# welcomyou/sherpa-vietnamese-asr

Measured on AMD Instinct MI355X. Metric: audio-sec/sec (xRT) Zipformer-68M offline decode, higher is better.
Workload: dtype bf16; 1 GPU; zipformer-68m greedy_search, batched planner chunks, 1 h per GPU; model=zipformer-68m, weights=greedy-calibrated, chunks_per_gpu=121, batch_pipeline=True, encoder_frames_per_gpu=98813

## Files before the change

include/zasr.h:

```cpp
#ifndef ZASR_H_
#define ZASR_H_

#include <stdint.h>

#ifdef __cplusplus
extern "C" {
#endif

typedef struct zasr_recognizer zasr_recognizer;
typedef struct zasr_result zasr_result;

enum {
  ZASR_OK = 0,
  ZASR_ERR_INVALID = 1,
  ZASR_ERR_NOT_FOUND = 2,
  ZASR_ERR_RUNTIME = 3,
};

enum {
  ZASR_PRECISION_FP32 = 0,
  ZASR_PRECISION_BF16 = 1,
  ZASR_PRECISION_BF16_ENC = 2,
  ZASR_PRECISION_BF16X3 = 3,
  ZASR_PRECISION_BF16X6 = 4,
// ... 106 lines not shown
void zasr_vad_destroy(zasr_vad* h);
int zasr_vad_probs(zasr_vad* h, const float* audio, const int64_t* offsets,
                   const int64_t* lengths, int32_t n_files, int32_t auto_boost, float* probs);
int zasr_vad_probs_device(zasr_vad* h, const float* d_audio, const int64_t* offsets,
                          const int64_t* lengths, int32_t n_files, int32_t auto_boost,
                          float* d_probs, void* stream);
int32_t zasr_vad_last_passes(const zasr_vad* h);
int zasr_vad_window(zasr_vad* h, const float* input, const float* state, int32_t n, float* prob,
                    float* state_out);

int32_t zasr_vocab_size(const zasr_recognizer* h);
int32_t zasr_joiner_dim(const zasr_recognizer* h);
int zasr_model_routes(zasr_recognizer* h, char* buf, int64_t cap);
int zasr_fbank_set_mel_banks(zasr_recognizer* h, const float* banks, int32_t n_bins);
int zasr_selftest_launch(int32_t block_threads);
int zasr_selftest_gemm_h3r(int32_t M, int32_t K, int32_t N, int32_t epi, const float* A,
                           const float* W, const float* bias, float* C);
int zasr_selftest_ffn_h3(int32_t R, int32_t D, int32_t F, const float* Y, const float* W1,
                         const float* b1, const float* W2, const float* b2,
                         const float* byp_orig, const float* byp_scale, float* X);
int zasr_selftest_ffn_bf16(int32_t R, int32_t D, int32_t F, const float* W1, const float* b1,
                           const float* W2, const float* b2, const float* byp_orig,
                           const float* byp_scale, float* X, int32_t form);

int zasr_profile_enable(zasr_recognizer* h, int32_t on);
int zasr_profile_reset(zasr_recognizer* h);
int zasr_profile_report(zasr_recognizer* h, char* buf, int64_t cap);

const char* zasr_last_error(void);
const char* zasr_version(void);

#ifdef __cplusplus
}
#endif
#endif
```

sherpa-vietnamese-asr_amd/csrc/attn_kernels.hip:

```cpp
#include <mutex>
#include <string>
#include <type_traits>
#include <unordered_map>

#include "common.h"
#include "gemm.h"
#include "gemm_dev.h"
#include "kernels.h"

namespace zasr {


namespace {
constexpr int kKLd = 40;
constexpr int kPosPad = 160;

__device__ __forceinline__ float fexp2(float x) { return __builtin_amdgcn_exp2f(x); }

typedef float f32x2 __attribute__((ext_vector_type(2)));
typedef __bf16 bf16x2 __attribute__((ext_vector_type(2)));
__device__ __forceinline__ f32x2 pk_fma(f32x2 a, f32x2 b, f32x2 c) { return __builtin_elementwise_fma(a, b, c); }

typedef _Float16 f16x8a __attribute__((ext_vector_type(8)));
typedef _Float16 f16x2 __attribute__((ext_vector_type(2)));
__device__ __forceinline__ void mfma_h3s(const bf16x8 (&x)[2], const f16x8a& ys, const f16x8a& yh,
                                         const f16x8a& yl, f32x16& acc) {
// ... 18 lines not shown
    lp[q / 2] = lo;
  }
  ys = __builtin_bit_cast(f16x8a, sp);
  yl = __builtin_bit_cast(f16x8a, lp);
  const _Float16 k = (_Float16)(1.f / 2048.f);
  yh = ys * (f16x8a){k, k, k, k, k, k, k, k};
}

}

template <int MODE, int NP, int FMT = 0, int NF = 1>
__global__ __launch_bounds__(256) void attn_flash_kernel(AttnFlashArgs a) {
  constexpr bool SPLIT = NP > 1;
  constexpr bool P1 = FMT == 1;
  static_assert(FMT == 0 || NP == 2, "fp16 pieces: NP = 2");
  static_assert(MODE != 3 || NP == 1 || (NP == 2 && FMT == 1),
                "fused NonlinAttention: the bf16 and f16x3 modes");
  constexpr bool W0 = MODE == 0 || MODE == 3;
  using T = typename std::conditional<SPLIT, float, __bf16>::type;
  extern __shared__ float sPos[];
  __shared__ __attribute__((aligned(16))) __bf16 sK[NP][2][32 * kKLd];
  __shared__ __attribute__((aligned(16))) __bf16 sVt[NP][2][12 * kKLd];
  __shared__ __attribute__((aligned(16))) __bf16 sVn[NP][2][MODE == 3 ? NF * 32 * kKLd : 8];
  const int b = blockIdx.y;
  const int h = W0 ? 0 : blockIdx.z;
  const int fz = MODE == 3 ? blockIdx.z : 0;
  const int r0 = a.row_off[b];
  const int L = a.row_off[b + 1] - r0;
  const int i0b = blockIdx.x * 128;
  if (i0b >= L) return;
  const int H = a.H;
  const long ldq = 68L * H;
  const long ldv = 12L * H;
  const T* qkp = reinterpret_cast<const T*>(a.qkp);
  const int tid = threadIdx.x, lane = tid & 63, wid = tid >> 6;
  const int c = lane & 31, h2 = lane >> 5;
  const int i0 = i0b + 32 * wid;
  const bool live = i0 < L;
  const int i = i0 + c;
  const int ic = i < L ? i : L - 1;
  constexpr float kSc = SPLIT ? 1.4426950408889634f : 1.f;
  constexpr float kE = P1 ? 11.f : 0.f;

  {
    const int xlo = -(i0b + 127);
    const int n = L + kPosPad;
    const int rmax = 2 * a.pmax - 2;
    for (int t = tid; t < n; t += 256) {
      int row = xlo + t + a.pmax - 1;
      row = row < 0 ? 0 : (row > rmax ? rmax : row);
      const float4 v = *reinterpret_cast<const float4*>(a.pos_tab + (long)row * 4 * H + 4 * h);
      if constexpr (SPLIT) {
        sPos[t] = v.x;
// ... 483 lines not shown
  static std::mutex mu;
  static std::unordered_map<const void*, size_t> memo;
  std::lock_guard<std::mutex> g(mu);
  auto it = memo.find(fn);
  if (it != memo.end()) return it->second;
  hipFuncAttributes at{};
  ZASR_HIP_CHECK(hipFuncGetAttributes(&at, fn));
  return memo[fn] = at.sharedSizeBytes;
}

template <int MODE, int NP, int FMT, int NF>
static void launch_flash_one(const AttnFlashArgs& a, dim3 grid, size_t lds, hipStream_t st) {
  const void* fn = reinterpret_cast<const void*>(&attn_flash_kernel<MODE, NP, FMT, NF>);
  const size_t stat = kernel_static_lds(fn);
  if (lds + stat > kLdsPerCu)
    throw std::runtime_error("attention: sequence of " + std::to_string(a.max_len) +
                             " frames needs " + std::to_string(lds + stat) +
                             " B of LDS (positional stage + static staging), over the " +
                             std::to_string(kLdsPerCu) + " B of a gfx950 CU");
  ZASR_LAUNCH((attn_flash_kernel<MODE, NP, FMT, NF>), grid, dim3(256), lds, st, a);
}

template <int NP, int FMT = 0>
void launch_flash_np(const AttnFlashArgs& a, int mode, size_t lds, hipStream_t st) {
  const dim3 grid(cdiv(a.max_len, 128), a.nseq, mode == 0 ? 1 : a.H);
  if (mode == 0)
    launch_flash_one<0, NP, FMT, 1>(a, grid, lds, st);
  else if (mode == 1)
    launch_flash_one<1, NP, FMT, 1>(a, grid, lds, st);
  else
    launch_flash_one<2, NP, FMT, 1>(a, grid, lds, st);
}

void launch_attn_flash(const AttnFlashArgs& a, int mode, hipStream_t st) {
  if (a.nseq <= 0 || a.max_len <= 0) return;
  if (mode == 3) {
    ZASR_REQUIRE((a.pieces == 1 || a.pieces == kPiecesF16) && a.t1t && a.o8 && a.y && a.z &&
                     a.hid > 0 && a.hid % 4 == 0 && a.ldt % 8 == 0 && a.ldy % 4 == 0,
                 "attention mode 3: the bf16 or f16x3 mode, hid % 4 == 0");
    const size_t lds = (size_t)(a.max_len + kPosPad) * sizeof(float4);
    const int nft = cdiv(a.hid, 32);
    if (a.pieces == kPiecesF16) {
      const dim3 grid(cdiv(a.max_len, 128), a.nseq, cdiv(nft, 3));
      launch_flash_one<3, 2, 1, 3>(a, grid, lds, st);
      return;
    }
    const int nf = (nft % 5 == 0 || nft == 9) ? 5 : 6;
    const dim3 grid(cdiv(a.max_len, 128), a.nseq, cdiv(nft, nf));
    if (nf == 5)
      launch_flash_one<3, 1, 0, 5>(a, grid, lds, st);
    else
      launch_flash_one<3, 1, 0, 6>(a, grid, lds, st);
    return;
  }
  ZASR_REQUIRE(a.H % 2 == 0, "attention: the bf16 kernels need an even head count (16-byte q/k rows)");
  const size_t lds = (size_t)(a.max_len + kPosPad) * sizeof(float4);
  if (a.pieces == 1)
    launch_flash_np<1>(a, mode, lds, st);
  else if (a.pieces == 2)
    launch_flash_np<2>(a, mode, lds, st);
  else if (a.pieces == 3)
    launch_flash_np<3>(a, mode, lds, st);
  else if (a.pieces == kPiecesF16)
    launch_flash_np<2, 1>(a, mode, lds, st);
  else
    throw std::runtime_error("attention: pieces must be 1, 2, 3 or kPiecesF16");
}

__device__ __forceinline__ float4 h3_load4(const float* p) { return *reinterpret_cast<const float4*>(p); }
__device__ __forceinline__ float4 h3_load4(const __bf16* p) {
  const bf16x4 v = *reinterpret_cast<const bf16x4*>(p);
  return make_float4((float)v[0], (float)v[1], (float)v[2], (float)v[3]);
}

template <typename TH, int NP>
__global__ __launch_bounds__(256) void nonlin_prep_t_kernel(const TH* __restrict__ h3,
                                                            const int* __restrict__ off,
                                                            const int* __restrict__ o8,
                                                            const int* __restrict__ map, int R,
                                                            int hid, int R8,
                                                            __bf16* __restrict__ t1t) {
  __shared__ float tile[64][65];
  __shared__ int sRow[64];
  const int col0 = blockIdx.x * 64, c0 = blockIdx.y * 64;
  const int tid = threadIdx.x;
  if (tid < 64) {
    const int col = col0 + tid;
    int lo = 0, hi = map[R - 1];
    while (lo < hi) {
// ... 99 lines not shown
```

sherpa-vietnamese-asr_amd/csrc/engine.cpp:

```cpp
#include "engine.h"

#include <algorithm>
#include <cmath>
#include <cstring>
#include <deque>
#include <numeric>
#include <cstdlib>
#include <sstream>

#include "common.h"
#include "gemm.h"
#include "host_io.h"
#include "onnx_io.h"

namespace zasr {

namespace {
struct HwNode {
  int tok = -1;
  double tok_score = 0, node_score = 0, out_score = 0;
  bool is_end = false;
  std::vector<std::pair<int, int>> kids;
  int fail = 0, out = -1;
  int child(int t) const {
// ... 961 lines not shown
  m.len = len;
  m.off.assign(len.size() + 1, 0);
  for (size_t b = 0; b < len.size(); ++b) {
    m.off[b + 1] = m.off[b] + len[b];
    m.maxlen = std::max(m.maxlen, len[b]);
  }
  m.total = m.off.back();
  return m;
}
struct MetaPack {
  std::vector<char> bytes;
  size_t add(const void* p, size_t n) {
    size_t at = (bytes.size() + 15) & ~size_t(15);
    bytes.resize(at + n);
    if (n) std::memcpy(bytes.data() + at, p, n);
    return at;
  }
};
}

void Engine::layer_forward(const DStack& S, const DLayer& Ly, float* X, int R, const int* d_off,
                           const int* d_map,
                           const std::vector<int>& lens, const long* d_aoff,
                           const void* d_slices_nl, int maxL, const int* d_o8, int R8, bool orig_ready, bool last_layer) {
  const int d = S.d, h = S.h, B = (int)lens.size();
  const int hid = 3 * d / 4;
  float* O = ws<float>("ly_orig", (size_t)R * d);
  if (!orig_ready)
    ZASR_HIP_CHECK(hipMemcpyAsync(O, X, (size_t)R * d * sizeof(float), hipMemcpyDeviceToDevice, st_));
  const bool bf16 = precision_ == 1 || precision_ == 2;
  const int np = split_pieces();
  float* qkp = nullptr;
  float* A = nullptr;
  __bf16* A16 = nullptr;
  float* stats = nullptr;
  AttnFlashArgs fa{};
  if (bf16) {
    __bf16* qkp16 = ws<__bf16>("ly_qkp_h", (size_t)R * 68 * h);
    linear_h(Ly.attn_in, X, false, d, R, qkp16, true, 68 * h, EPI_NONE);
    A16 = ws<__bf16>("ly_attn_h", 1);
    stats = ws<float>("ly_attn_stats", (size_t)R * h);
    fa = AttnFlashArgs{qkp16, h, Ly.pos_tab, model_.pmax, d_off, d_aoff, B, maxL, A16,
                       nullptr, nullptr, stats, stats};
  } else if (np) {
    qkp = ws<float>("ly_qkp", (size_t)R * 68 * h);
    linear(Ly.attn_in, X, d, R, qkp, 68 * h, EPI_NONE);
    A = ws<float>("ly_attn", 1);
    stats = ws<float>("ly_attn_stats", (size_t)R * h);
    fa = AttnFlashArgs{qkp, h, Ly.pos_tab, model_.pmax, d_off, d_aoff, B, maxL, A,
                       nullptr, nullptr, stats, stats, np};
    if (np != kPiecesF16) {
      prof_begin("attn_softmax");
      launch_attn_flash(fa, 0, st_);
      prof_end();
    }
  } else {
    qkp = ws<float>("ly_qkp", (size_t)R * 68 * h);
    linear(Ly.attn_in, X, d, R, qkp, 68 * h, EPI_NONE);
    A = ws<float>("ly_attn", 1);
    stats = ws<float>("ly_attn_stats", (size_t)R * h * 2);
    AttnArgs a{qkp, h, Ly.pos_tab, model_.pmax, d_off, d_aoff, B, maxL, A, stats, 1};
    prof_begin("attn_softmax");
    launch_attn_softmax(a, st_);
    prof_end();
  }
  auto ff = [&](int k) {
    const DLin& fi = Ly.ff_in[k];
    const float* bo = (bf16 && k == 1) ? O : nullptr;
    const float* bs = (bf16 && k == 1) ? Ly.bypass_mid : nullptr;
    if (fi.wh && ffn_fused_supported(d) && (d < 256 || fi.wp)) {
      prof_begin("ffn_fused");
      launch_ffn_fused(X, R, d, fi.N, d < 256 ? fi.wh : fi.wp, fi.b,
                       d < 256 ? Ly.ff_out[k].wh : Ly.ff_out[k].wp, Ly.ff_out[k].b, st_, bo, bs);
      prof_end();
      return;
    }
// ... 2 lines not shown
      linear_h(fi, X, false, d, R, H, true, fi.N, EPI_SWOOSHL);
      linear_h(Ly.ff_out[k], H, true, fi.N, R, X, false, d, EPI_RESADD, bo, bs);
    } else if (fi.wp && np == kPiecesF16) {
      prof_begin("ffn_fused");
      launch_ffn_fused_h3(X, R, d, fi.N, fi.wp, fi.b, Ly.ff_out[k].wp, Ly.ff_out[k].b, st_,
                          k == 1 ? O : nullptr, k == 1 ? Ly.bypass_mid : nullptr);
      prof_end();
    } else {
      const bool byp = k == 1 && Ly.ff_out[k].wx != nullptr;
      float* H = ws<float>("ly_hid", (size_t)R * fi.N);
      linear(fi, X, d, R, H, fi.N, EPI_SWOOSHL);
      linear(Ly.ff_out[k], H, fi.N, R, X, d, EPI_RESADD, "enc_gemm", byp ? O : nullptr,
             byp ? Ly.bypass_mid : nullptr);
    }
  };
  auto self_attn = [&](int k) {
    if (bf16) {
      __bf16* vv = ws<__bf16>("ly_vv_h", (size_t)R * 12 * h);
      __bf16* oa = ws<__bf16>("ly_oa_h", (size_t)R * 12 * h);
      linear_h(Ly.sa_in[k], X, false, d, R, vv, true, 12 * h, EPI_NONE);
      AttnFlashArgs a = fa;
      a.v = vv;
      a.out = oa;
      prof_begin("attn_apply");
      launch_attn_flash(a, k == 0 ? 1 : 2, st_);
      prof_end();
      linear_h(Ly.sa_out[k], oa, true, 12 * h, R, X, false, d, EPI_RESADD);
      return;
    }
    float* vv = ws<float>("ly_vv", (size_t)R * 12 * h);
    float* oa = ws<float>("ly_oa", (size_t)R * 12 * h);
    linear(Ly.sa_in[k], X, d, R, vv, 12 * h, EPI_NONE);
    if (np) {
      AttnFlashArgs a = fa;
      a.v = vv;
      a.out = oa;
      prof_begin("attn_apply");
      launch_attn_flash(a, k == 0 ? 1 : 2, st_);
      prof_end();
      linear(Ly.sa_out[k], oa, 12 * h, R, X, d, EPI_RESADD);
      return;
    }
    AttnSAArgs sa{qkp, h, Ly.pos_tab, model_.pmax, d_off, B, maxL, stats, vv, oa, stats};
    prof_begin("attn_apply");
    launch_attn_sa(sa, k == 0, false, st_);
    prof_end();
    linear(Ly.sa_out[k], oa, 12 * h, R, X, d, EPI_RESADD);
  };
  auto conv = [&](int k) {
    if (Ly.cv_in[k].wh) {
      __bf16* dc = ws<__bf16>("ly_dc_h", (size_t)R * d);
      if (Ly.cv_in[k].glu) {
        __bf16* g = ws<__bf16>("ly_glu_h", (size_t)R * d);
        linear_h(Ly.cv_in[k], X, false, d, R, g, true, d, EPI_GLU);
        prof_begin("dwconv1d");
        launch_dwconv1d_post_glu_bf16(g, d_off, d_map, R, d, S.K, Ly.cv_dw_w[k], Ly.cv_dw_b[k], dc, st_);
        prof_end();
      } else {
        __bf16* g2 = ws<__bf16>("ly_g2_h", (size_t)R * 2 * d);
// ... 18 lines not shown
      prof_begin("dwconv1d");
      launch_glu_dwconv1d(g2, d_off, d_map, R, d, S.K, Ly.cv_dw_w[k], Ly.cv_dw_b[k], dc, st_);
      prof_end();
    }
    linear(Ly.cv_out[k], dc, d, R, X, d, EPI_RESADD);
  };
  ff(0);
  if (bf16) {
    __bf16* h3 = ws<__bf16>("ly_h3_h", (size_t)R * 3 * hid);
    __bf16* t1t = ws<__bf16>("ly_t1t", (size_t)hid * R8);
    __bf16* z = ws<__bf16>("ly_z_h", (size_t)R * hid);
    linear_h(Ly.na_in, X, false, d, R, h3, true, 3 * hid, EPI_NONE);
    prof_begin("elementwise");
    launch_nonlin_prep_t(h3, true, d_off, d_o8, d_map, R, hid, R8, t1t, st_);
    prof_end();
    AttnFlashArgs a = fa;
    a.t1t = t1t;
    a.o8 = d_o8;
    a.ldt = R8;
    a.hid = hid;
    a.y = h3 + 2 * hid;
    a.ldy = 3 * hid;
    a.z = z;
    prof_begin("attn_nonlin");
    launch_attn_flash(a, 3, st_);
    prof_end();
    linear_h(Ly.na_out, z, true, hid, R, X, false, d, EPI_RESADD);
  } else if (np) {
    float* h3 = ws<float>("ly_h3", (size_t)R * 3 * hid);
    __bf16* t1t = ws<__bf16>("ly_t1t_x", (size_t)stored_pieces(np) * hid * R8);
    float* z = ws<float>("ly_z", (size_t)R * hid);
    linear(Ly.na_in, X, d, R, h3, 3 * hid, EPI_NONE);
    prof_begin("elementwise");
    launch_nonlin_prep_t(h3, false, d_off, d_o8, d_map, R, hid, R8, t1t, st_, np);
    prof_end();
    if (np == kPiecesF16) {
      AttnFlashArgs a = fa;
      a.t1t = t1t;
      a.o8 = d_o8;
      a.ldt = R8;
      a.hid = hid;
      a.y = h3 + 2 * hid;
      a.ldy = 3 * hid;
      a.z = z;
      prof_begin("attn_nonlin");
      launch_attn_flash(a, 3, st_);
      prof_end();
    } else {
    GemmParams p{};
    p.A = A;
    p.B = nullptr;
    p.sbk = 1;
    p.sbn = R8;
    p.C = z;
    p.ldc = hid;
    p.N = hid;
    p.alpha = 1.f;
    p.aux = h3 + 2 * hid;
    p.ldaux = 3 * hid;
    p.slices = reinterpret_cast<const GemmSlice*>(d_slices_nl);
    p.num_slices = B;
    p.max_M = maxL;
    prof_begin("attn_nonlin");
    gemm_x3(p, t1t, (long)hid * R8, EPI_MULAUX, ALOAD_DENSE, st_, np);
    prof_end();
    }
    linear(Ly.na_out, z, hid, R, X, d, EPI_RESADD);
// ... 86 lines not shown
      g.aux_off = (long)mst[i].off[b] * 3 * hid;
      g.M = Lb;
      g.K = flash ? L8 : Lb;
      g.lda = Lp;
      sl_nl[i].push_back(g);
      acc += (long)Lb * Lp;
      c8 += L8;
    }
    o8[i].push_back(c8);
    R8[i] = c8;
    attn_floats = std::max(attn_floats, (size_t)acc);
  }
  ensure_pos_tables(maxL_all + 192);
  std::vector<GemmSlice> sl_c2(B), sl_c3(B);
  for (int b = 0; b < B; ++b) {
    sl_c2[b] = GemmSlice{(long)mc1.off[b] * 640, 0, (long)mc2.off[b] * 39 * 32, 0, l2[b] * 39, 72, 0, 0};
    sl_c3[b] = GemmSlice{(long)mc2.off[b] * 39 * 32, 0, (long)mL.off[b] * 19 * 128, 0, L[b] * 19, 288, 0, 0};
  }
  MetaPack mp;
  size_t o_fb = mp.add(mfb.off.data(), (B + 1) * 4), o_c1 = mp.add(mc1.off.data(), (B + 1) * 4),
         o_L = mp.add(mL.off.data(), (B + 1) * 4), o_out = mp.add(mout.off.data(), (B + 1) * 4);
  size_t o_c2s = mp.add(sl_c2.data(), B * sizeof(GemmSlice)),
         o_c3s = mp.add(sl_c3.data(), B * sizeof(GemmSlice));
  std::vector<size_t> o_st(ns), o_ao(ns), o_sn(ns), o_o8(ns);
  for (int i = 0; i < ns; ++i) {
    o_st[i] = mp.add(mst[i].off.data(), (B + 1) * 4);
    o_o8[i] = mp.add(o8[i].data(), (B + 1) * 4);
    o_ao[i] = mp.add(aoff[i].data(), B * sizeof(long));
    o_sn[i] = mp.add(sl_nl[i].data(), sl_nl[i].size() * sizeof(GemmSlice));
  }
  char* d_meta = ws<char>("enc_meta", mp.bytes.size());
  upload(d_meta, mp.bytes.data(), mp.bytes.size());
  auto I = [&](size_t o) { return reinterpret_cast<const int*>(d_meta + o); };
  int* c1_map = ws<int>("map_c1", mc1.total);
  int* L_map = ws<int>("map_L", mL.total);
  int* out_map = ws<int>("map_out", mout.total);
  launch_row2seq(I(o_c1), B, mc1.total, c1_map, st_);
  launch_row2seq(I(o_L), B, mL.total, L_map, st_);
  launch_row2seq(I(o_out), B, mout.total, out_map, st_);
  std::vector<int*> st_map(ns);
  for (int i = 0; i < ns; ++i) {
    st_map[i] = ws<int>("map_st" + std::to_string(i), mst[i].total);
    launch_row2seq(I(o_st[i]), B, mst[i].total, st_map[i], st_);
  }

  const bool fe16 = model_.conv4.wh != nullptr && model_.conv7.wh != nullptr;
  void* c1 = fe16 ? (void*)ws<__bf16>("fe_c1_h", (size_t)mc1.total * 640)
                  : (void*)ws<float>("fe_c1", (size_t)mc1.total * 640);
  prof_begin("frontend_conv");
  launch_conv1(d_feats, I(o_fb), I(o_c1), c1_map, mc1.total, model_.conv0_w, model_.conv0_b, c1,
               fe16, st_, split_pieces() == kPiecesF16);
  prof_end();
// ... 93 lines not shown
    ws<float>("ly_attn", split_pieces() == kPiecesF16 ? 1 : std::max<size_t>(attn_floats, 1));
  const int Dm = cfg.max_dim();
  float* full = ws<float>("st_full", (size_t)mL.total * Dm);
  float* orig = ws<float>("st_orig0", (size_t)mL.total * model_.stacks[0].d);
  prof_begin("elementwise");
  launch_copy_cols(e0, d0, 0, orig, model_.stacks[0].d, 0, std::min(d0, model_.stacks[0].d),
                   mL.total, true, model_.stacks[0].d, st_);
  prof_end();
  for (int i = 0; i < ns; ++i) {
    const DStack& s = model_.stacks[i];
    const int d = s.d;
    float* X;
    if (s.ds == 1) {
      X = orig;
    } else {
      X = ws<float>("st_x", (size_t)mst[i].total * d);
      prof_begin("elementwise");
      launch_downsample(orig, I(o_L), I(o_st[i]), st_map[i], mst[i].total, d, s.ds, s.ds_w, X, st_);
      prof_end();
    }
    for (size_t li = 0; li < s.layers.size(); ++li)
      layer_forward(s, s.layers[li], X, mst[i].total, I(o_st[i]), st_map[i], mst[i].len,
                    reinterpret_cast<const long*>(d_meta + o_ao[i]), d_meta + o_sn[i],
                    mst[i].maxlen, I(o_o8[i]), R8[i], li > 0, li + 1 == s.layers.size());
    int later_max = 0;
    for (int j = i + 1; j < ns; ++j) later_max = std::max(later_max, model_.stacks[j].d);
    const int dn = i + 1 < ns ? model_.stacks[i + 1].d : 0;
    float* next = i + 1 < ns ? ws<float>("st_orig" + std::to_string((i + 1) % 2), (size_t)mL.total * dn)
                             : nullptr;
    prof_begin("elementwise");
    launch_stack_glue(X, orig, I(o_L), I(o_st[i]), L_map, mL.total, d, s.ds, s.comb, next, dn,
                      d > later_max ? full : nullptr, Dm, later_max, st_);
    prof_end();
    orig = next;
  }
  float* fo = ws<float>("enc_ds", (size_t)mout.total * Dm);
  prof_begin("elementwise");
  launch_downsample(full, I(o_L), I(o_out), out_map, mout.total, Dm, 2, model_.out_ds_w, fo, st_);
  prof_end();
  linear(model_.enc_proj, fo, Dm, mout.total, d_enc, cfg.joiner_dim, EPI_NONE);
}

std::vector<TokenResult> Engine::run_search(const float* d_enc, const std::vector<int>& t_out,
                                            int beam) {
  SearchJob job;
  launch_search(d_enc, t_out, beam, 0, st_, true, job);
  return collect_search(job);
// ... 683 lines not shown
```

sherpa-vietnamese-asr_amd/csrc/engine.h:

```cpp
#pragma once
#include <hip/hip_runtime.h>

#include <map>
#include <mutex>
#include <string>
#include <vector>

#include "gemm.h"
#include "kernels.h"

namespace zasr {

struct ModelConfig {
  std::string name;
  std::vector<int> dims, layers, ff, heads, ds, kernels;
  int qd = 32, vd = 12, pd = 4, pos_dim = 48;
  int V = 0, dec_dim = 0, joiner_dim = 0, context = 2;
  int c1 = 8, c2 = 32, c3 = 128;
  int max_dim() const {
    int m = 0;
    for (int d : dims) m = d > m ? d : m;
    return m;
  }
};
// ... 141 lines not shown
  void pin_reset(int arena);

  void run_fbank(const float* d_wav, const std::vector<long>& wav_off, const std::vector<long>& n,
                 float* d_feats, std::vector<int>& frames);
  void run_encoder(const float* d_feats, const std::vector<int>& T, float* d_enc,
                   std::vector<int>& t_out);
  std::vector<TokenResult> run_search(const float* d_enc, const std::vector<int>& t_out, int beam);
  struct SearchJob {
    int S_all = 0, S = 0, cap = 0, set = 0, Tmax = 0;
    std::vector<int> order, t_out;
    bool check_finite = false;
    hipStream_t stream = nullptr;
  };
  void launch_search(const float* d_enc, const std::vector<int>& t_out, int beam, int set,
                     hipStream_t stream, bool split_groups, SearchJob& job);
  std::vector<TokenResult> collect_search(SearchJob& job);
  struct ResPin {
    char* p = nullptr;
    size_t cap = 0;
  };
  ResPin res_pin_[kMaxJobs];
  void layer_forward(const DStack& stk, const DLayer& ly, float* X, int R, const int* d_off,
                     const int* d_map, const std::vector<int>& lens, const long* d_aoff,
                     const void* d_slices_nl, int maxL, const int* d_o8, int R8, bool orig_ready = false,
                     bool last_layer = true);
  void linear(const DLin& l, const float* A, int lda, int M, float* C, int ldc, int epi,
              const char* cls = "enc_gemm", const float* byp_orig = nullptr,
              const float* byp_scale = nullptr);
  void linear_h(const DLin& l, const void* A, bool a_bf16, int lda, int M, void* C, bool c_bf16,
                int ldc, int epi, const float* byp_orig = nullptr,
                const float* byp_scale = nullptr);
  void ensure_pos_tables(int max_len);

  struct ProfEvent {
    std::string name;
    hipEvent_t a, b;
  };
  void prof_begin(const char* name);
  void prof_begin(const std::string& name);
  void prof_end();
  static std::string shape_key(const char* cls, int M, int K, int N, bool w16, bool a16,
                               bool c16, int epi);
  bool prof_on_ = false;
  bool prof_shapes_ = false;
  std::vector<ProfEvent> prof_pending_;
  std::map<std::string, std::pair<long, double>> prof_acc_;
  std::vector<hipEvent_t> event_pool_;
// ... 39 lines not shown
```

sherpa-vietnamese-asr_amd/csrc/kernels.h:

```cpp
#pragma once
#include <cstdint>

#include <hip/hip_runtime.h>

namespace zasr {

struct FbankTables {
  const double* twiddle;
  const float* window;
  const int* mel_start;
  const int* mel_len;
  const int* mel_woff;
  const float* mel_w;
};
void launch_fbank(const float* wav, const long* wav_off, const int* nsamp, const int* fr_off,
                  int nseq, int total_frames, const FbankTables& tabs, float* out,
                  hipStream_t st, bool campp = false);

void launch_silence_flags(const float* wav, long n, int frame_len, float threshold,
                          unsigned char* flags, hipStream_t st);

void launch_selftest_noop(int block_threads);
void selftest_gemm_h3r(int M, int K, int N, int epi, const float* A, const float* W,
                       const float* bias, float* C);
// ... 156 lines not shown
void launch_attn_softmax(const AttnArgs& a, hipStream_t st);
struct AttnFlashArgs {
  const void* qkp;
  int H;
  const float* pos_tab;
  int pmax;
  const int* row_off;
  const long* a_off;
  int nseq;
  int max_len;
  void* attn;
  const void* v;
  void* out;
  const float* stats_in;
  float* stats_out;
  int pieces = 1;
  const void* t1t = nullptr;
  const int* o8 = nullptr;
  int ldt = 0;
  int hid = 0;
  const void* y = nullptr;
  int ldy = 0;
  void* z = nullptr;
};
void launch_attn_flash(const AttnFlashArgs& a, int mode, hipStream_t st);
void launch_nonlin_prep_t(const void* h3, bool h3_bf16, const int* off, const int* o8,
                          const int* map, int R, int hid, int R8, void* t1t, hipStream_t st,
                          int pieces = 1);
struct AttnSAArgs {
  const float* qkp;
  int H;
  const float* pos_tab;
  int pmax;
  const int* row_off;
  int nseq;
  int max_len;
  const float* stats;
  const float* v;
  float* out;
  float* stats_out;
};
void launch_attn_sa(const AttnSAArgs& a, bool online, bool bf16, hipStream_t st);

bool ffn_fused_supported(int D);
void ffn_pack_host(const __bf16* w, int rows, int cols, __bf16* out);
void launch_ffn_fused(float* X, int R, int D, int F, const void* W1, const float* b1,
                      const void* W2, const float* b2, hipStream_t st,
                      const float* byp_orig = nullptr, const float* byp_scale = nullptr);
// ... 139 lines not shown
```

sherpa-vietnamese-asr_amd/csrc/zasr_api.cpp:

```cpp
#include <cstdio>
#include <cstring>
#include <fstream>
#include <memory>
#include <mutex>
#include <sstream>
#include <string>
#include <vector>

#include "../../include/zasr.h"
#include "campp.h"
#include "common.h"
#include "vad.h"
#include "vibert.h"
#include "engine.h"
#include "host_io.h"
#include "onnx_io.h"

using zasr::Engine;
using zasr::TokenResult;

struct zasr_recognizer {
  std::unique_ptr<Engine> eng;
  std::string model_dir;
  std::string tokens_path;
// ... 635 lines not shown
  });
}

int zasr_selftest_ffn_h3(int32_t R, int32_t D, int32_t F, const float* Y, const float* W1,
                         const float* b1, const float* W2, const float* b2,
                         const float* byp_orig, const float* byp_scale, float* X) {
  if (!Y || !W1 || !b1 || !W2 || !b2 || !X) return fail(ZASR_ERR_INVALID, "null argument");
  return guarded([&]() {
    zasr::selftest_ffn_h3(R, D, F, Y, W1, b1, W2, b2, byp_orig, byp_scale, X);
    return (int)ZASR_OK;
  });
}

int zasr_selftest_ffn_bf16(int32_t R, int32_t D, int32_t F, const float* W1, const float* b1,
                           const float* W2, const float* b2, const float* byp_orig,
                           const float* byp_scale, float* X, int32_t form) {
  if (!W1 || !b1 || !W2 || !b2 || !X) return fail(ZASR_ERR_INVALID, "null argument");
  return guarded([&]() {
    zasr::selftest_ffn_bf16(R, D, F, W1, b1, W2, b2, byp_orig, byp_scale, X, form);
    return (int)ZASR_OK;
  });
}

int zasr_silence_flags(const float* d_wav, int64_t n, int32_t frame_len, float threshold,
                       uint8_t* d_flags, void* stream) {
  if (n < 0 || (n > 0 && (!d_wav || !d_flags))) return fail(ZASR_ERR_INVALID, "null argument");
  return guarded([&]() {
    zasr::launch_silence_flags(d_wav, (long)n, (int)frame_len, threshold, d_flags,
                               reinterpret_cast<hipStream_t>(stream));
    return (int)ZASR_OK;
  });
}

int zasr_set_tokens(zasr_recognizer* h, const char* tokens_path) {
  if (!h || !tokens_path) return fail(ZASR_ERR_INVALID, "null argument");
  return guarded([&]() {
    std::ifstream f(tokens_path);
    if (!f) return fail(ZASR_ERR_NOT_FOUND, std::string("tokens file not found: ") + tokens_path);
    std::lock_guard<std::mutex> lk(h->sym_mu);
    h->tokens_path = tokens_path;
    h->syms.reset();
    return (int)ZASR_OK;
  });
}

int zasr_create_stream(zasr_recognizer* h, zasr_stream** out) {
// ... 98 lines not shown
```

sherpa-vietnamese-asr_amd/zasr/binding.py:

```python
from __future__ import annotations

import ctypes as C
import dataclasses
import os
from typing import List, Optional, Sequence

import numpy as np

_PKG = os.path.dirname(os.path.dirname(os.path.abspath(__file__)))
DEFAULT_LIB = os.path.join(_PKG, "lib", "libzasr.so")

EXPORTS = (
    "zasr_create", "zasr_destroy", "zasr_convert_model", "zasr_convert_stage_model", "zasr_fbank", "zasr_decode_batch", "zasr_decode_features",
    "zasr_decode_device", "zasr_decode_device_batches", "zasr_encode_features", "zasr_search_encoder_out",
    "zasr_result_count", "zasr_result_num_tokens", "zasr_result_num_frames",
    "zasr_result_tokens", "zasr_result_frames", "zasr_result_log_probs",
    "zasr_result_token_stats", "zasr_result_free", "zasr_vocab_size", "zasr_joiner_dim",
    "zasr_profile_enable", "zasr_profile_reset", "zasr_profile_report", "zasr_last_error",
    "zasr_version", "zasr_campp_create", "zasr_campp_destroy", "zasr_campp_embedding_dim",
    "zasr_campp_fbank", "zasr_campp_embed", "zasr_campp_embed_device", "zasr_campp_windows_device",
    "zasr_vibert_create", "zasr_vibert_destroy", "zasr_vibert_num_labels",
    "zasr_vibert_num_detect", "zasr_vibert_run",
    "zasr_vad_create", "zasr_vad_destroy", "zasr_vad_probs", "zasr_vad_probs_device",
    "zasr_vad_window", "zasr_vad_last_passes", "zasr_silence_flags",
    "zasr_create_stream", "zasr_destroy_stream", "zasr_stream_accept_waveform",
    "zasr_decode_stream", "zasr_decode_streams", "zasr_stream_is_decoded",
    "zasr_stream_num_tokens", "zasr_stream_num_frames", "zasr_stream_tokens",
    "zasr_stream_frames", "zasr_stream_log_probs", "zasr_stream_token_stats",
    "zasr_stream_result_json", "zasr_set_tokens", "zasr_model_routes",
    "zasr_fbank_set_mel_banks", "zasr_selftest_launch", "zasr_decode_host_batches",
    "zasr_selftest_gemm_h3r", "zasr_selftest_ffn_h3", "zasr_selftest_ffn_bf16",
)


PRECISIONS = {"fp32": 0, "bf16": 1, "bf16_enc": 2, "bf16x3": 3, "bf16x6": 4, "f16x3": 5}


C_FP = C.POINTER(C.c_float)


class ZasrError(RuntimeError):
    pass


class _Config(C.Structure):
    _fields_ = [
        ("model_dir", C.c_char_p),
        ("decoding_method", C.c_char_p),
        ("max_active_paths", C.c_int32),
        ("blank_penalty", C.c_float),
        ("hotword_tokens", C.POINTER(C.c_int32)),
        ("hotword_lens", C.POINTER(C.c_int32)),
        ("hotword_scores", C.POINTER(C.c_float)),
        ("num_hotwords", C.c_int32),
# ... 132 lines not shown
    lib.zasr_stream_tokens.restype = C.POINTER(I32)
    lib.zasr_stream_frames.argtypes = [P]
    lib.zasr_stream_frames.restype = C.POINTER(I32)
    lib.zasr_stream_log_probs.argtypes = [P]
    lib.zasr_stream_log_probs.restype = C.POINTER(C.c_double)
    lib.zasr_stream_token_stats.argtypes = [P]
    lib.zasr_stream_token_stats.restype = fp
    lib.zasr_stream_result_json.argtypes = [P, C.c_char_p, I64, C.POINTER(I64)]
    lib.zasr_stream_result_json.restype = C.c_int
    lib.zasr_set_tokens.argtypes = [P, C.c_char_p]
    lib.zasr_set_tokens.restype = C.c_int
    lib.zasr_model_routes.argtypes = [P, C.c_char_p, I64]
    lib.zasr_model_routes.restype = C.c_int
    lib.zasr_fbank_set_mel_banks.argtypes = [P, fp, I32]
    lib.zasr_fbank_set_mel_banks.restype = C.c_int
    lib.zasr_selftest_launch.argtypes = [I32]
    lib.zasr_selftest_launch.restype = C.c_int
    lib.zasr_selftest_gemm_h3r.argtypes = [I32, I32, I32, I32, fp, fp, fp, fp]
    lib.zasr_selftest_gemm_h3r.restype = C.c_int
    lib.zasr_selftest_ffn_h3.argtypes = [I32, I32, I32, fp, fp, fp, fp, fp, fp, fp, fp]
    lib.zasr_selftest_ffn_h3.restype = C.c_int
    lib.zasr_selftest_ffn_bf16.argtypes = [I32, I32, I32, fp, fp, fp, fp, fp, fp, fp, I32]
    lib.zasr_selftest_ffn_bf16.restype = C.c_int
    if path is None:
        _lib = lib
    return lib


def convert_model(model_dir: str, out_dir: str, lib_path: Optional[str] = None) -> None:
    lib = load_library(lib_path)
    os.makedirs(out_dir, exist_ok=True)
    rc = lib.zasr_convert_model(model_dir.encode(), out_dir.encode())
    if rc != 0:
        msg = lib.zasr_last_error().decode()
        if rc == 2:
            raise FileNotFoundError(msg)
        raise ZasrError(msg)


def convert_stage_model(kind: str, model_dir: str, out_dir: str,
                        lib_path: Optional[str] = None) -> None:
    lib = load_library(lib_path)
    os.makedirs(out_dir, exist_ok=True)
    rc = lib.zasr_convert_stage_model(kind.encode(), model_dir.encode(), out_dir.encode())
    if rc != 0:
        msg = lib.zasr_last_error().decode()
# ... 29 lines not shown
    bo = None if byp_orig is None else _f32(byp_orig)
    bs = None if byp_scale is None else _f32(byp_scale)
    p = lambda x: None if x is None else x.ctypes.data_as(C_FP)
    rc = lib.zasr_selftest_ffn_h3(Y.shape[0], Y.shape[1], W1.shape[0], p(Y), p(W1), p(b1), p(W2),
                                  p(b2), p(bo), p(bs), p(X))
    if rc != 0:
        raise ZasrError(lib.zasr_last_error().decode())
    return X


def selftest_ffn_bf16(W1, b1, W2, b2, X, byp_orig=None, byp_scale=None, form: int = 0,
                      lib_path: Optional[str] = None) -> np.ndarray:
    lib = load_library(lib_path)
    W1, b1, W2, b2, X = (_f32(v) for v in (W1, b1, W2, b2, X))
    X = X.copy()
    bo = None if byp_orig is None else _f32(byp_orig)
    bs = None if byp_scale is None else _f32(byp_scale)
    p = lambda x: None if x is None else x.ctypes.data_as(C_FP)
    rc = lib.zasr_selftest_ffn_bf16(X.shape[0], X.shape[1], W1.shape[0], p(W1), p(b1), p(W2),
                                    p(b2), p(bo), p(bs), p(X), int(form))
    if rc != 0:
        raise ZasrError(lib.zasr_last_error().decode())
    return X


def silence_flags(d_wav_ptr: int, n: int, frame_len: int, threshold: float, d_flags_ptr: int,
                  stream: int = 0, lib_path: Optional[str] = None) -> None:
    lib = load_library(lib_path)
    rc = lib.zasr_silence_flags(C.c_void_p(d_wav_ptr), int(n), int(frame_len),
                                float(threshold), C.c_void_p(d_flags_ptr), C.c_void_p(stream))
    if rc != 0:
        raise ZasrError(lib.zasr_last_error().decode())


@dataclasses.dataclass
class SearchResult:
    token_ids: np.ndarray
    frames: np.ndarray
    log_probs: np.ndarray
    stats: np.ndarray
    T: int


def _f32(a) -> np.ndarray:
    return np.ascontiguousarray(np.asarray(a, dtype=np.float32))

# ... 438 lines not shown
```

Baseline: 128,200 audio-sec/sec.

## Schedule flash-attention blocks through a host-built XCD-balanced block map

The flash attention kernels switch from a 3D grid of (tiles, sequences, heads) to a 1D grid indexed through a packed block map built on the host. The map drops empty tiles past each sequence's length and spreads work, weighted by tile count times key length, evenly over the 8 XCDs via round-robin slot interleaving. Consecutive heads of one sequence stay on the same XCD, which should improve L2 reuse of K/V, and idle blocks from the padded max_len grid go away. In exchange it adds host-side map construction and upload per batch, plus bit-field limits on sequence count, heads and tiles.

```diff
diff --git a/include/zasr.h b/include/zasr.h
--- a/include/zasr.h
+++ b/include/zasr.h
@@ -152,6 +152,8 @@
 int zasr_selftest_ffn_bf16(int32_t R, int32_t D, int32_t F, const float* W1, const float* b1,
                            const float* W2, const float* b2, const float* byp_orig,
                            const float* byp_scale, float* X, int32_t form);
+int zasr_selftest_attn_block_map(const int32_t* lens, int32_t nseq, int32_t units_per_seq,
+                                 int32_t order, uint32_t* out, int64_t cap, int32_t* grid);
 
 int zasr_profile_enable(zasr_recognizer* h, int32_t on);
 int zasr_profile_reset(zasr_recognizer* h);
diff --git a/sherpa-vietnamese-asr_amd/csrc/attn_kernels.hip b/sherpa-vietnamese-asr_amd/csrc/attn_kernels.hip
--- a/sherpa-vietnamese-asr_amd/csrc/attn_kernels.hip
+++ b/sherpa-vietnamese-asr_amd/csrc/attn_kernels.hip
@@ -1,7 +1,9 @@
+#include <algorithm>
 #include <mutex>
 #include <string>
 #include <type_traits>
 #include <unordered_map>
+#include <vector>
 
 #include "common.h"
 #include "gemm.h"
@@ -66,13 +68,15 @@
   __shared__ __attribute__((aligned(16))) __bf16 sK[NP][2][32 * kKLd];
   __shared__ __attribute__((aligned(16))) __bf16 sVt[NP][2][12 * kKLd];
   __shared__ __attribute__((aligned(16))) __bf16 sVn[NP][2][MODE == 3 ? NF * 32 * kKLd : 8];
-  const int b = blockIdx.y;
-  const int h = W0 ? 0 : blockIdx.z;
-  const int fz = MODE == 3 ? blockIdx.z : 0;
+  const unsigned ent = a.map[blockIdx.x];
+  if (ent == kAttnMapNone) return;
+  const int b = ent >> 12;
+  const int unit = (ent >> 8) & 15;
+  const int h = W0 ? 0 : unit;
+  const int fz = MODE == 3 ? unit : 0;
   const int r0 = a.row_off[b];
   const int L = a.row_off[b + 1] - r0;
-  const int i0b = blockIdx.x * 128;
-  if (i0b >= L) return;
+  const int i0b = (ent & 255) * 128;
   const int H = a.H;
   const long ldq = 68L * H;
   const long ldv = 12L * H;
@@ -602,8 +606,7 @@
 }
 
 template <int NP, int FMT = 0>
-void launch_flash_np(const AttnFlashArgs& a, int mode, size_t lds, hipStream_t st) {
-  const dim3 grid(cdiv(a.max_len, 128), a.nseq, mode == 0 ? 1 : a.H);
+void launch_flash_np(const AttnFlashArgs& a, int mode, dim3 grid, size_t lds, hipStream_t st) {
   if (mode == 0)
     launch_flash_one<0, NP, FMT, 1>(a, grid, lds, st);
   else if (mode == 1)
@@ -614,37 +617,90 @@
 
 void launch_attn_flash(const AttnFlashArgs& a, int mode, hipStream_t st) {
   if (a.nseq <= 0 || a.max_len <= 0) return;
+  ZASR_REQUIRE(a.map && a.map_len > 0 && a.map_len % kAttnXcds == 0,
+               "attention: no block map (build_attn_block_map)");
+  ZASR_REQUIRE(a.max_len <= 128 * kAttnMapMaxTiles && a.nseq <= kAttnMapMaxSeq,
+               "attention: sequence count or length over the block map's fields");
+  const dim3 grid(a.map_len);
   if (mode == 3) {
     ZASR_REQUIRE((a.pieces == 1 || a.pieces == kPiecesF16) && a.t1t && a.o8 && a.y && a.z &&
                      a.hid > 0 && a.hid % 4 == 0 && a.ldt % 8 == 0 && a.ldy % 4 == 0,
                  "attention mode 3: the bf16 or f16x3 mode, hid % 4 == 0");
     const size_t lds = (size_t)(a.max_len + kPosPad) * sizeof(float4);
-    const int nft = cdiv(a.hid, 32);
     if (a.pieces == kPiecesF16) {
-      const dim3 grid(cdiv(a.max_len, 128), a.nseq, cdiv(nft, 3));
       launch_flash_one<3, 2, 1, 3>(a, grid, lds, st);
       return;
     }
-    const int nf = (nft % 5 == 0 || nft == 9) ? 5 : 6;
-    const dim3 grid(cdiv(a.max_len, 128), a.nseq, cdiv(nft, nf));
-    if (nf == 5)
+    if (attn_nonlin_frags(a.hid, a.pieces) == 5)
       launch_flash_one<3, 1, 0, 5>(a, grid, lds, st);
     else
       launch_flash_one<3, 1, 0, 6>(a, grid, lds, st);
     return;
   }
   ZASR_REQUIRE(a.H % 2 == 0, "attention: the bf16 kernels need an even head count (16-byte q/k rows)");
+  ZASR_REQUIRE(a.H <= kAttnMapMaxUnits, "attention: head count over the block map's field");
   const size_t lds = (size_t)(a.max_len + kPosPad) * sizeof(float4);
   if (a.pieces == 1)
-    launch_flash_np<1>(a, mode, lds, st);
+    launch_flash_np<1>(a, mode, grid, lds, st);
   else if (a.pieces == 2)
-    launch_flash_np<2>(a, mode, lds, st);
+    launch_flash_np<2>(a, mode, grid, lds, st);
   else if (a.pieces == 3)
-    launch_flash_np<3>(a, mode, lds, st);
+    launch_flash_np<3>(a, mode, grid, lds, st);
   else if (a.pieces == kPiecesF16)
-    launch_flash_np<2, 1>(a, mode, lds, st);
+    launch_flash_np<2, 1>(a, mode, grid, lds, st);
   else
     throw std::runtime_error("attention: pieces must be 1, 2, 3 or kPiecesF16");
+}
+
+int build_attn_block_map(const int* lens, int nseq, int units, int order, std::vector<unsigned>& map) {
+  ZASR_REQUIRE(nseq >= 0 && nseq <= kAttnMapMaxSeq && units >= 1 && units <= kAttnMapMaxUnits &&
+                   (order == 0 || order == 1),
+               "attention block map: sequences, units per sequence or slot order out of range");
+  auto tiles = [](int L) { return (L + 127) / 128; };
+  auto weight = [&](int L) { return (long)tiles(L) * ((L + 31) / 32); };
+  long total = 0;
+  for (int b = 0; b < nseq; ++b) {
+    ZASR_REQUIRE(lens[b] >= 0 && tiles(lens[b]) <= kAttnMapMaxTiles,
+                 "attention block map: sequence length out of range");
+    total += weight(lens[b]) * units;
+  }
+  map.clear();
+  if (total == 0) return 0;
+  struct Run {
+    int seq, u0, n;
+  };
+  std::vector<Run> runs[kAttnXcds];
+  long before = 0;
+  for (int b = 0; b < nseq; ++b) {
+    const long w = weight(lens[b]);
+    if (w == 0) continue;
+    for (int u = 0; u < units; ++u, before += w) {
+      const int x = (int)((2 * before + w) * kAttnXcds / (2 * total));
+      if (!runs[x].empty() && runs[x].back().seq == b)
+        ++runs[x].back().n;
+      else
+        runs[x].push_back(Run{b, u, 1});
+    }
+  }
+  long slots = 0;
+  for (const auto& rs : runs) {
+    long n = 0;
+    for (const Run& r : rs) n += (long)r.n * tiles(lens[r.seq]);
+    slots = std::max(slots, n);
+  }
+  ZASR_REQUIRE(slots * kAttnXcds <= INT32_MAX, "attention block map: too many blocks");
+  map.assign((size_t)slots * kAttnXcds, kAttnMapNone);
+  for (int x = 0; x < kAttnXcds; ++x) {
+    size_t slot = 0;
+    for (const Run& r : runs[x]) {
+      const int nt = tiles(lens[r.seq]);
+      for (int e = 0; e < nt * r.n; ++e) {
+        const int t = order == 0 ? e / r.n : e % nt, u = r.u0 + (order == 0 ? e % r.n : e / nt);
+        map[kAttnXcds * slot++ + x] = attn_map_pack(r.seq, u, t);
+      }
+    }
+  }
+  return (int)map.size();
 }
 
 __device__ __forceinline__ float4 h3_load4(const float* p) { return *reinterpret_cast<const float4*>(p); }
diff --git a/sherpa-vietnamese-asr_amd/csrc/engine.cpp b/sherpa-vietnamese-asr_amd/csrc/engine.cpp
--- a/sherpa-vietnamese-asr_amd/csrc/engine.cpp
+++ b/sherpa-vietnamese-asr_amd/csrc/engine.cpp
@@ -1007,7 +1007,8 @@
 void Engine::layer_forward(const DStack& S, const DLayer& Ly, float* X, int R, const int* d_off,
                            const int* d_map,
                            const std::vector<int>& lens, const long* d_aoff,
-                           const void* d_slices_nl, int maxL, const int* d_o8, int R8, bool orig_ready, bool last_layer) {
+                           const void* d_slices_nl, int maxL, const int* d_o8, int R8,
+                           const AttnBlockMaps& bm, bool orig_ready, bool last_layer) {
   const int d = S.d, h = S.h, B = (int)lens.size();
   const int hid = 3 * d / 4;
   float* O = ws<float>("ly_orig", (size_t)R * d);
@@ -1035,8 +1036,11 @@
     fa = AttnFlashArgs{qkp, h, Ly.pos_tab, model_.pmax, d_off, d_aoff, B, maxL, A,
                        nullptr, nullptr, stats, stats, np};
     if (np != kPiecesF16) {
+      AttnFlashArgs a = fa;
+      a.map = bm.head0;
+      a.map_len = bm.n_head0;
       prof_begin("attn_softmax");
-      launch_attn_flash(fa, 0, st_);
+      launch_attn_flash(a, 0, st_);
       prof_end();
     }
   } else {
@@ -1085,6 +1089,8 @@
       AttnFlashArgs a = fa;
       a.v = vv;
       a.out = oa;
+      a.map = bm.heads;
+      a.map_len = bm.n_heads;
       prof_begin("attn_apply");
       launch_attn_flash(a, k == 0 ? 1 : 2, st_);
       prof_end();
@@ -1098,6 +1104,8 @@
       AttnFlashArgs a = fa;
       a.v = vv;
       a.out = oa;
+      a.map = bm.heads;
+      a.map_len = bm.n_heads;
       prof_begin("attn_apply");
       launch_attn_flash(a, k == 0 ? 1 : 2, st_);
       prof_end();
@@ -1162,6 +1170,8 @@
     a.y = h3 + 2 * hid;
     a.ldy = 3 * hid;
     a.z = z;
+    a.map = bm.head0;
+    a.map_len = bm.n_head0;
     prof_begin("attn_nonlin");
     launch_attn_flash(a, 3, st_);
     prof_end();
@@ -1183,6 +1193,8 @@
       a.y = h3 + 2 * hid;
       a.ldy = 3 * hid;
       a.z = z;
+      a.map = bm.head0;
+      a.map_len = bm.n_head0;
       prof_begin("attn_nonlin");
       launch_attn_flash(a, 3, st_);
       prof_end();
@@ -1315,12 +1327,25 @@
          o_L = mp.add(mL.off.data(), (B + 1) * 4), o_out = mp.add(mout.off.data(), (B + 1) * 4);
   size_t o_c2s = mp.add(sl_c2.data(), B * sizeof(GemmSlice)),
          o_c3s = mp.add(sl_c3.data(), B * sizeof(GemmSlice));
-  std::vector<size_t> o_st(ns), o_ao(ns), o_sn(ns), o_o8(ns);
+  std::vector<size_t> o_st(ns), o_ao(ns), o_sn(ns), o_o8(ns), o_bmh(ns), o_bm0(ns);
+  std::vector<int> n_bmh(ns, 0), n_bm0(ns, 0);
+  std::vector<unsigned> bmap;
   for (int i = 0; i < ns; ++i) {
     o_st[i] = mp.add(mst[i].off.data(), (B + 1) * 4);
     o_o8[i] = mp.add(o8[i].data(), (B + 1) * 4);
     o_ao[i] = mp.add(aoff[i].data(), B * sizeof(long));
     o_sn[i] = mp.add(sl_nl[i].data(), sl_nl[i].size() * sizeof(GemmSlice));
+    if (flash) {
+      const DStack& s = model_.stacks[i];
+      const int np = split_pieces();
+      const bool fused_nl = bf16 || np == kPiecesF16;
+      n_bmh[i] = build_attn_block_map(mst[i].len.data(), B, s.h, 0, bmap);
+      o_bmh[i] = mp.add(bmap.data(), bmap.size() * sizeof(unsigned));
+      n_bm0[i] = build_attn_block_map(mst[i].len.data(), B,
+                                      fused_nl ? attn_nonlin_chunks(3 * s.d / 4, bf16 ? 1 : np) : 1,
+                                      0, bmap);
+      o_bm0[i] = mp.add(bmap.data(), bmap.size() * sizeof(unsigned));
+    }
   }
   char* d_meta = ws<char>("enc_meta", mp.bytes.size());
   upload(d_meta, mp.bytes.data(), mp.bytes.size());
@@ -1460,7 +1485,10 @@
     for (size_t li = 0; li < s.layers.size(); ++li)
       layer_forward(s, s.layers[li], X, mst[i].total, I(o_st[i]), st_map[i], mst[i].len,
                     reinterpret_cast<const long*>(d_meta + o_ao[i]), d_meta + o_sn[i],
-                    mst[i].maxlen, I(o_o8[i]), R8[i], li > 0, li + 1 == s.layers.size());
+                    mst[i].maxlen, I(o_o8[i]), R8[i],
+                    AttnBlockMaps{reinterpret_cast<const unsigned*>(d_meta + o_bmh[i]), n_bmh[i],
+                                  reinterpret_cast<const unsigned*>(d_meta + o_bm0[i]), n_bm0[i]},
+                    li > 0, li + 1 == s.layers.size());
     int later_max = 0;
     for (int j = i + 1; j < ns; ++j) later_max = std::max(later_max, model_.stacks[j].d);
     const int dn = i + 1 < ns ? model_.stacks[i + 1].d : 0;
diff --git a/sherpa-vietnamese-asr_amd/csrc/engine.h b/sherpa-vietnamese-asr_amd/csrc/engine.h
--- a/sherpa-vietnamese-asr_amd/csrc/engine.h
+++ b/sherpa-vietnamese-asr_amd/csrc/engine.h
@@ -187,7 +187,8 @@
   ResPin res_pin_[kMaxJobs];
   void layer_forward(const DStack& stk, const DLayer& ly, float* X, int R, const int* d_off,
                      const int* d_map, const std::vector<int>& lens, const long* d_aoff,
-                     const void* d_slices_nl, int maxL, const int* d_o8, int R8, bool orig_ready = false,
+                     const void* d_slices_nl, int maxL, const int* d_o8, int R8,
+                     const AttnBlockMaps& bm, bool orig_ready = false,
                      bool last_layer = true);
   void linear(const DLin& l, const float* A, int lda, int M, float* C, int ldc, int epi,
               const char* cls = "enc_gemm", const float* byp_orig = nullptr,
diff --git a/sherpa-vietnamese-asr_amd/csrc/kernels.h b/sherpa-vietnamese-asr_amd/csrc/kernels.h
--- a/sherpa-vietnamese-asr_amd/csrc/kernels.h
+++ b/sherpa-vietnamese-asr_amd/csrc/kernels.h
@@ -1,5 +1,6 @@
 #pragma once
 #include <cstdint>
+#include <vector>
 
 #include <hip/hip_runtime.h>
 
@@ -202,8 +203,33 @@
   const void* y = nullptr;
   int ldy = 0;
   void* z = nullptr;
+  const unsigned* map = nullptr;
+  int map_len = 0;
 };
 void launch_attn_flash(const AttnFlashArgs& a, int mode, hipStream_t st);
+inline int attn_nonlin_frags(int hid, int pieces) {
+  const int nft = (hid + 31) / 32;
+  if (pieces != 1) return 3;
+  return (nft % 5 == 0 || nft == 9) ? 5 : 6;
+}
+inline int attn_nonlin_chunks(int hid, int pieces) {
+  const int nf = attn_nonlin_frags(hid, pieces);
+  return ((hid + 31) / 32 + nf - 1) / nf;
+}
+constexpr int kAttnXcds = 8;
+constexpr unsigned kAttnMapNone = 0xffffffffu;
+constexpr int kAttnMapMaxSeq = 1 << 20, kAttnMapMaxUnits = 16, kAttnMapMaxTiles = 256;
+inline unsigned attn_map_pack(int seq, int unit, int tile) {
+  return (unsigned)seq << 12 | (unsigned)unit << 8 | (unsigned)tile;
+}
+struct AttnBlockMaps {
+  const unsigned* heads;
+  int n_heads;
+  const unsigned* head0;
+  int n_head0;
+};
+int build_attn_block_map(const int* lens, int nseq, int units_per_seq, int order,
+                         std::vector<unsigned>& map);
 void launch_nonlin_prep_t(const void* h3, bool h3_bf16, const int* off, const int* o8,
                           const int* map, int R, int hid, int R8, void* t1t, hipStream_t st,
                           int pieces = 1);
diff --git a/sherpa-vietnamese-asr_amd/csrc/zasr_api.cpp b/sherpa-vietnamese-asr_amd/csrc/zasr_api.cpp
--- a/sherpa-vietnamese-asr_amd/csrc/zasr_api.cpp
+++ b/sherpa-vietnamese-asr_amd/csrc/zasr_api.cpp
@@ -681,6 +681,18 @@
   });
 }
 
+int zasr_selftest_attn_block_map(const int32_t* lens, int32_t nseq, int32_t units_per_seq,
+                                 int32_t order, uint32_t* out, int64_t cap, int32_t* grid) {
+  if (!lens || !grid || (cap > 0 && !out) || cap < 0) return fail(ZASR_ERR_INVALID, "null argument");
+  return guarded([&]() {
+    std::vector<unsigned> map;
+    *grid = zasr::build_attn_block_map(lens, nseq, units_per_seq, order, map);
+    if ((int64_t)map.size() > cap) return fail(ZASR_ERR_INVALID, "block map buffer too small");
+    std::copy(map.begin(), map.end(), out);
+    return (int)ZASR_OK;
+  });
+}
+
 int zasr_silence_flags(const float* d_wav, int64_t n, int32_t frame_len, float threshold,
                        uint8_t* d_flags, void* stream) {
   if (n < 0 || (n > 0 && (!d_wav || !d_flags))) return fail(ZASR_ERR_INVALID, "null argument");
diff --git a/sherpa-vietnamese-asr_amd/zasr/binding.py b/sherpa-vietnamese-asr_amd/zasr/binding.py
--- a/sherpa-vietnamese-asr_amd/zasr/binding.py
+++ b/sherpa-vietnamese-asr_amd/zasr/binding.py
@@ -30,6 +30,7 @@
     "zasr_stream_result_json", "zasr_set_tokens", "zasr_model_routes",
     "zasr_fbank_set_mel_banks", "zasr_selftest_launch", "zasr_decode_host_batches",
     "zasr_selftest_gemm_h3r", "zasr_selftest_ffn_h3", "zasr_selftest_ffn_bf16",
+    "zasr_selftest_attn_block_map",
 )
 
 
@@ -208,6 +209,9 @@
     lib.zasr_selftest_ffn_h3.restype = C.c_int
     lib.zasr_selftest_ffn_bf16.argtypes = [I32, I32, I32, fp, fp, fp, fp, fp, fp, fp, I32]
     lib.zasr_selftest_ffn_bf16.restype = C.c_int
+    lib.zasr_selftest_attn_block_map.argtypes = [C.POINTER(I32), I32, I32, I32,
+                                                 C.POINTER(C.c_uint32), I64, C.POINTER(I32)]
+    lib.zasr_selftest_attn_block_map.restype = C.c_int
     if path is None:
         _lib = lib
     return lib
@@ -283,6 +287,22 @@
     if rc != 0:
         raise ZasrError(lib.zasr_last_error().decode())
     return X
+
+
+def selftest_attn_block_map(lens, units_per_seq: int, order: int = 0,
+                            lib_path: Optional[str] = None) -> np.ndarray:
+    lib = load_library(lib_path)
+    lens = np.ascontiguousarray(lens, dtype=np.int32)
+    cap = 8 * int(units_per_seq) * int(((lens.astype(np.int64) + 127) // 128).sum())
+    out = np.empty(max(cap, 1), dtype=np.uint32)
+    grid = C.c_int32(-1)
+    rc = lib.zasr_selftest_attn_block_map(lens.ctypes.data_as(C.POINTER(C.c_int32)), len(lens),
+                                          int(units_per_seq), int(order),
+                                          out.ctypes.data_as(C.POINTER(C.c_uint32)), cap,
+                                          C.byref(grid))
+    if rc != 0:
+        raise ZasrError(lib.zasr_last_error().decode())
+    return out[:grid.value].copy()
 
 
 def silence_flags(d_wav_ptr: int, n: int, frame_len: int, threshold: float, d_flags_ptr: int,
```

Result: faster. 131,000 audio-sec/sec, median of 6 (+2.2%).
